# RinceWND/extPOM

Hardware: AMD Instinct MI355X
Metric: 3D cell-updates/sec on internal mode (one internal step = the 3-D baroclinic step and its isplit 2-D external substeps; whole-step wall time) (higher is better)
Workload: dtype f64

## Files before the change

### extpom_amd/csrc/k_vert.hip

```cpp
#include <type_traits>
#include "pomgpu_internal.hpp"
#include "dd_exp.h"

#define dt_(i, j) F2(dt, i, j)
#define dx_(i, j) F2(dx, i, j)
#define dy_(i, j) F2(dy, i, j)
#define h_(i, j) F2(h, i, j)
#define u_(i, j, k) F3(u, i, j, k)
#define v_(i, j, k) F3(v, i, j, k)
#define w_(i, j, k) F3(w, i, j, k)

#define ROWS_PROFUV 1
#define ROWS_PROFT 1
#ifndef ROWS_UVF
#define ROWS_UVF 8
#endif
#ifndef ROWS_UVM
#define ROWS_UVM 4
#endif
#define COL2                               \
  const int i = TID_I, j = TID_J;          \
  if (i > P.iml || j > P.jml) return;

__global__ void k_baropg(KP P, int sum2d) {
// ... 1148 lines not shown
    km_c = km_n;
    if (k + 2 <= kb) km_n = KMA(k + 2);
  }
  const double tps = 0.5 * (F2(cbc, i, j) + F2(cbc, i, j - 1)) *
                     sqrt(sq(.25 * (F3(ub, i, j, kbm1) + F3(ub, i + 1, j, kbm1) + F3(ub, i, j - 1, kbm1) + F3(ub, i + 1, j - 1, kbm1))) +
                          sq(F3(vb, i, j, kbm1)));
  const double c = -P.dti2 * (KMA(kbm1) + P.umol) / (F1(dz, kbm1) * F1(dzz, kbm2) * dh * dh);
  const double m = F2(dvm, i, j);
  double x = (c * gg[kbm2 - 1] - rhs_k) / (tps * P.dti2 / (-F1(dz, kbm1) * dh) - 1. - (ee[kbm2 - 1] - 1.) * c);
  x = x * m;
  F3(vf, i, j, kbm1) = x;
  F2(wvbot, i, j) = -tps * x;
  for (int ki = kbm2; ki >= 1; ki--) {
    x = (ee[ki - 1] * x + gg[ki - 1]) * m;
    F3(vf, i, j, ki) = x;
  }
  if (do_adv) F3(vf, i, j, kb) = 0.;
  F2(tps, i, j) = tps;
#undef RHS
#undef VFLUX
#undef KMA
}

template <int KBT, int V>
static __device__ __forceinline__ void d_profuv_reg(const KP &P, const bool store_tps) {
  const int j = TID_J;
  if (j > P.jm) return;
  int i0, lane = 1;
  if (V) { i0 = TID_I; } else { lane = HALO_LANE; i0 = HALO_COL; }
  const bool out = (lane >= 1 && lane <= 62 && i0 >= 2 && i0 <= P.imm1 && j >= 2 && j <= P.jmm1);
#ifdef POMGPU_EMU
  if (!out) return;
#else
  if (V && !out) return;
  if (j < 2 || j > P.jmm1) return;
#endif
  const int i = i0 < 1 ? 1 : (i0 > P.iml ? P.iml : i0);
  const int iw = i > 1 ? i - 1 : 1, js = j > 1 ? j - 1 : 1;
  const int in_ = V ? i : iw, jn_ = V ? js : j;
  double *f = P.b3 + (size_t)(V ? P3_vf : P3_uf) * P.a3;
  const unsigned col = POMGPU_ST_BYTES * (unsigned)((j - 1) * P.iml + (i - 1)), col2 = POMGPU_ST_BYTES * (unsigned)((js - 1) * P.iml + (i - 1));
  const double *kmp = P.b3 + (size_t)P3_km * P.a3;
#define PLANE(ptr, k, off) REF3((pomgpu_st *)((char *)((pomgpu_st *)(ptr) + (size_t)((k)-1) * P.n2) + (off)), 0)
  const int kb = P.kb, kbm1 = P.kbm1, kbm2 = P.kbm2;
  double ee[KBT], gg[KBT];
#define KC(k) ((k) < kbm1 ? (k) : kbm1)
#define KCB(k) ((k) < kb ? (k) : kb)
#pragma unroll
  for (int k = 1; k <= KBT; k++) ee[k - 1] = PLANE(kmp, KCB(k), col);
  if (V) {
#pragma unroll
    for (int k = 1; k <= KBT; k++) gg[k - 1] = PLANE(kmp, KCB(k), col2);
  } else {
#pragma unroll
    for (int k = 1; k <= KBT - 1; k++) gg[k - 1] = PLANE(f, KC(k), col);
  }
  const double rhs_b = G3(f, i, j, kbm1);
  const double dh = V ? .5 * (F2(h, i, j) + F2(etf, i, j) + F2(h, i, js) + F2(etf, i, js))
                      : (F2(h, i, j) + F2(etf, i, j) + F2(h, iw, j) + F2(etf, iw, j)) * .5;
  const double wsurf = V ? F2(wvsurf, i, j) : F2(wusurf, i, j);
  const double m = V ? F2(dvm, i, j) : F2(dum, i, j);
  const double cb2 = F2(cbc, i, j) + F2(cbc, in_, jn_);
  double tps;
  if (V) tps = 0.5 * cb2 * sqrt(sq(.25 * (F3(ub, i, j, kbm1) + F3(ub, i + 1, j, kbm1) + F3(ub, i, js, kbm1) + F3(ub, i + 1, js, kbm1))) +
                                sq(F3(vb, i, j, kbm1)));
  else tps = 0.5 * cb2 * sqrt(sq(F3(ub, i, j, kbm1)) +
                              sq(.25 * (F3(vb, i, j, kbm1) + F3(vb, i, j + 1, kbm1) + F3(vb, iw, j, kbm1) + F3(vb, iw, j + 1, kbm1))));
  SCHED_FENCE();
#pragma unroll
  for (int k = 1; k <= KBT; k++) {
    ee[k - 1] = (ee[k - 1] + (V ? gg[k - 1] : halo_w(ee[k - 1], [&] { return F3(km, iw, j, KCB(k)); }))) * .5;
    if (!V && (k & 3) == 0) SCHED_FENCE();
  }
  if (V) {
    SCHED_FENCE();
#pragma unroll
    for (int k = 1; k <= KBT - 1; k++) gg[k - 1] = PLANE(f, KC(k), col);
  }
  SCHED_FENCE();
#define KMA(k) ee[(k)-1]
  double km_c = KMA(1), km_n = KMA(2);
  double e_prev, g_prev;
  {
    const double a = -P.dti2 * (km_n + P.umol) / (F1(dz, 1) * F1(dzz, 1) * dh * dh);
    e_prev = a / (a - 1.);
    g_prev = (-P.dti2 * wsurf / (-F1(dz, 1) * dh) - gg[0]) / (a - 1.);
    ee[0] = e_prev; gg[0] = g_prev;
  }
  double e_last = e_prev, g_last = g_prev, km_last = km_n;
#pragma unroll
  for (int k = 2; k <= KBT - 2; k++) {
    km_c = km_n;
    km_n = KMA(k + 1);
    const double a = -P.dti2 * (km_n + P.umol) / (F1(dz, KC(k)) * F1(dzz, KC(k)) * dh * dh);
    const double c = -P.dti2 * (km_c + P.umol) / (F1(dz, KC(k)) * F1(dzz, KC(k - 1)) * dh * dh);
    const double g = 1. / (a + c * (1. - e_prev) - 1.);
    e_prev = a * g;
    g_prev = (c * g_prev - gg[k - 1]) * g;
    ee[k - 1] = e_prev; gg[k - 1] = g_prev;
    const bool fin = (k == kbm2);
    e_last = fin ? e_prev : e_last;
    g_last = fin ? g_prev : g_last;
    km_last = fin ? km_n : km_last;
  }
#undef KMA
  if (!out) return;
  const double c = -P.dti2 * (km_last + P.umol) / (F1(dz, kbm1) * F1(dzz, kbm2) * dh * dh);
  double x = (c * g_last - rhs_b) / (tps * P.dti2 / (-F1(dz, kbm1) * dh) - 1. - (e_last - 1.) * c);
  x = x * m;
  G3(f, i, j, kbm1) = x;
  if (V) F2(wvbot, i, j) = -tps * x; else F2(wubot, i, j) = -tps * x;
#pragma unroll
  for (int ki = KBT - 2; ki >= 1; ki--) {
    const double xn = (ee[ki - 1] * x + gg[ki - 1]) * m;
    if (ki <= kbm2) { x = xn; PLANE(f, ki, col) = x; }
  }
  if (store_tps) F2(tps, i, j) = tps;
#undef KC
#undef KCB
#undef PLANE
}
template <int KBT, int V>
__global__ void __launch_bounds__(64 * ROWS_PROFUV) k_profuv_reg(KP P) { d_profuv_reg<KBT, V>(P, true); }
template <int KBT>
__global__ void __launch_bounds__(64 * ROWS_PROFUV) k_profuv_reg2(KP P) {
  if (blockIdx.z == 0) d_profuv_reg<KBT, 0>(P, false);
  else d_profuv_reg<KBT, 1>(P, true);
}

#define UVF_GHOST(P, i, j) (((i) == 1 && !(P).W) || ((i) == (P).im && !(P).E) || ((j) == 1 && !(P).S) || ((j) == (P).jm && !(P).N))
__global__ void k_uv_filter(KP P, int own) {
  COL2
  if (own && UVF_GHOST(P, i, j)) return;
  const bool act = (i <= P.im && j <= P.jm);
  double su = 0., sv = 0.;
  if (act) {
    for (int k = 1; k <= P.kbm1; k++) {
      const double dzk = F1(dz, k);
      su = su + (F3(uf, i, j, k) + F3(ub, i, j, k) - 2. * F3(u, i, j, k)) * dzk;
      sv = sv + (F3(vf, i, j, k) + F3(vb, i, j, k) - 2. * F3(v, i, j, k)) * dzk;
    }
  }
  for (int k = 1; k <= P.kb; k++) {
    const double uf = F3(uf, i, j, k), vf = F3(vf, i, j, k);
    double u = F3(u, i, j, k), v = F3(v, i, j, k);
    if (act && k <= P.kbm1) {
      u = u + .5 * P.smoth * (uf + F3(ub, i, j, k) - 2. * u - su);
      v = v + .5 * P.smoth * (vf + F3(vb, i, j, k) - 2. * v - sv);
    }
    F3(ub, i, j, k) = u;
// ... 73 lines not shown
        dk[k - 1] = d;
        if (k <= kbm1) {
          su = su + d * F1(dz, k);
          G3(c, i, j, k) = uf;
        }
      }
    }
    SCHED_FENCE();
  }
#pragma unroll
  for (int k = 1; k <= NL; k++)
    if (k <= kbm1) G3(b, i, j, k) = uo[k - 1] + .5 * P.smoth * (dk[k - 1] - su);
  G3(b, i, j, kb) = c_kb;
  G3(c, i, j, kb) = f_kb;
  if (V) F2(tps, i, j) = su;
#undef KC
}
template <int KBT, int V>
__global__ void __launch_bounds__(64 * ROWS_UVF) k_uv_filter_reg(KP P, int own) { d_uv_filter_reg<KBT, V>(P, own); }
template <int KBT>
__global__ void __launch_bounds__(64 * ROWS_UVF) k_uv_filter_reg2(KP P, int own) {
  if (blockIdx.z == 0) d_uv_filter_reg<KBT, 0>(P, own);
  else d_uv_filter_reg<KBT, 1>(P, own);
}

static inline dim3 colblk() { return dim3(64, 2, 1); }
static inline dim3 rowblk(int rows) { return dim3(64, rows, 1); }
static inline dim3 rowgrid(const KP &P, int rows) { return dim3((P.iml + 63) / 64, (P.jml + rows - 1) / rows, 1); }
static inline dim3 colgrid(const KP &P) { return dim3((P.iml + 63) / 64, (P.jml + 1) / 2, 1); }
#define COLV_G(P) dim3(((P).iml + 63) / 64, ((P).jml + 3) / 4, 1)
#define COLV_B dim3(64, 4, 1)
void launch_baropg(pomgpu_ctx *c, int sum2d) {
  if (SW(c, BAROPG_CELLS)) { LAUNCH(c, k_baropg, COLV_G(c->P), COLV_B, c->P, sum2d); return; }
  LAUNCHN(c, "k_baropg", k_baropg_rs, grid1_halo_r(c->P, BPG_ROWS), blk_col_r(BPG_ROWS), c->P, sum2d);
}
void launch_baropg_mcc(pomgpu_ctx *c, int sum2d) { LAUNCH(c, k_baropg_mcc, colgrid(c->P), colblk(), c->P, sum2d); }
void launch_order_pack(pomgpu_ctx *c, double *send_e, double *send_n) {
  const KP &P = c->P;
  const int len = P.iml > P.jml ? P.iml : P.jml;
  LAUNCH(c, k_order_pack, dim3((len + 63) / 64, P.kb + 1, 1), dim3(64, 1, 1), c->P, send_e, send_n);
}
static inline dim3 twin(dim3 g) { g.z = 2; return g; }
template <int KBT> static void launch_int_uvmean_reg_t(pomgpu_ctx *c) {
  if (!SW(c, NO_TWIN)) { LAUNCHN(c, "k_int_uvmean_reg2", (k_int_uvmean_reg2<KBT>), twin(rowgrid(c->P, ROWS_UVM)), rowblk(ROWS_UVM), c->P); return; }
  LAUNCHN(c, "k_int_uvmean_reg", (k_int_uvmean_reg<KBT, 0>), rowgrid(c->P, ROWS_UVM), rowblk(ROWS_UVM), c->P);
  LAUNCHN(c, "k_int_uvmean_reg", (k_int_uvmean_reg<KBT, 1>), rowgrid(c->P, ROWS_UVM), rowblk(ROWS_UVM), c->P);
// ... 76 lines not shown
void launch_advu_profu(pomgpu_ctx *c, int do_adv, int do_prof) { LAUNCH(c, k_advu_profu, colgrid(c->P), colblk(), c->P, do_adv, do_prof); }
void launch_advv_profv(pomgpu_ctx *c, int do_adv, int do_prof) { LAUNCH(c, k_advv_profv, colgrid(c->P), colblk(), c->P, do_adv, do_prof); }
template <int KBT> static void launch_profuv_reg_t(pomgpu_ctx *c) {
  const KP &P = c->P;
  if (!SW(c, NO_TWIN)) {
    LAUNCHN(c, "k_profuv_reg2", (k_profuv_reg2<KBT>), dim3((P.iml + 61) / 62, (P.jml + ROWS_PROFUV - 1) / ROWS_PROFUV, 2), rowblk(ROWS_PROFUV), c->P);
    return;
  }
  LAUNCHN(c, "k_profu_reg", (k_profuv_reg<KBT, 0>), dim3((P.iml + 61) / 62, (P.jml + ROWS_PROFUV - 1) / ROWS_PROFUV, 1), rowblk(ROWS_PROFUV), c->P);
  LAUNCHN(c, "k_profv_reg", (k_profuv_reg<KBT, 1>), rowgrid(P, ROWS_PROFUV), rowblk(ROWS_PROFUV), c->P);
}
int launch_profuv_reg(pomgpu_ctx *c) {
  const int kb = c->P.kb;
  if (SW(c, THOMAS_SCRATCH) || kb > 64 || kb < 6) return 0;
  if (kb <= 24) launch_profuv_reg_t<24>(c);
  else if (kb <= 32) launch_profuv_reg_t<32>(c);
  else if (kb <= 40) launch_profuv_reg_t<40>(c);
  else if (kb <= 44) launch_profuv_reg_t<44>(c);
  else if (kb <= 50) launch_profuv_reg_t<50>(c);
  else if (kb <= 56) launch_profuv_reg_t<56>(c);
  else launch_profuv_reg_t<64>(c);
  return 1;
}
template <int KBT> static void launch_uv_filter_reg_t(pomgpu_ctx *c, int own) {
  if (!SW(c, NO_TWIN)) { LAUNCHN(c, "k_uv_filter_reg2", (k_uv_filter_reg2<KBT>), twin(rowgrid(c->P, ROWS_UVF)), rowblk(ROWS_UVF), c->P, own); return; }
  LAUNCHN(c, "k_uv_filter_reg", (k_uv_filter_reg<KBT, 0>), rowgrid(c->P, ROWS_UVF), rowblk(ROWS_UVF), c->P, own);
  LAUNCHN(c, "k_uv_filter_reg", (k_uv_filter_reg<KBT, 1>), rowgrid(c->P, ROWS_UVF), rowblk(ROWS_UVF), c->P, own);
}
static int launch_uv_filter_reg(pomgpu_ctx *c, int own) {
  const int kb = c->P.kb;
  if (SW(c, THOMAS_SCRATCH) || kb > 64 || kb < 6) return 0;
  if (kb <= 24) launch_uv_filter_reg_t<24>(c, own);
  else if (kb <= 32) launch_uv_filter_reg_t<32>(c, own);
  else if (kb <= 40) launch_uv_filter_reg_t<40>(c, own);
  else if (kb <= 44) launch_uv_filter_reg_t<44>(c, own);
  else if (kb <= 50) launch_uv_filter_reg_t<50>(c, own);
  else if (kb <= 56) launch_uv_filter_reg_t<56>(c, own);
  else launch_uv_filter_reg_t<64>(c, own);
  return 1;
}
void launch_uv_filter(pomgpu_ctx *c, int own) {
  if (launch_uv_filter_reg(c, own)) return;
  LAUNCH(c, k_uv_filter, colgrid(c->P), colblk(), c->P, own);
}
```

### extpom_amd/csrc/pomgpu_api.hip

```cpp
#include <math.h>
#include <stdarg.h>
#include <stdio.h>
#include <stdlib.h>
#include <string.h>
#include <vector>
#include "pomgpu.h"
#include "pomgpu_internal.hpp"

struct ProfPair { int slot; hipEvent_t a, b; };
struct ProfState { std::vector<ProfPair> pending; std::vector<ProfPair> free_; char filter[64]; };
static ProfState *PS(pomgpu_ctx *c) { return (ProfState *)c->prof_state; }

#define SLOT2(c, n) ((c)->P.b2 + (size_t)(n) * (c)->P.n2)
#define SLOT3(c, n) ((c)->P.b3 + (size_t)(n) * (c)->P.a3)
#define D2(c, name) SLOT2(c, P2_##name)
#define D3(c, name) SLOT3(c, P3_##name)
#define LEV3(c, p, lev) ((double *)((pomgpu_st *)(p) + (size_t)(lev) * (c)->P.n2))

int pomgpu_fail(pomgpu_ctx *c, int code, const char *fmt, ...) {
  if (c && c->parent) c = c->parent;
  if (c) {
    va_list ap;
    va_start(ap, fmt);
    vsnprintf(c->err, sizeof c->err, fmt, ap);
// ... 177 lines not shown
static void ext_buffers(pomgpu_ctx *c) {
  KP &P = c->P;
  for (int n = 0; n < POMGPU_NGEN; n++) P.x2[n] = P.y2[n] = c->ext_parity ? c->alt2[n] : P.b2 + (size_t)X2_SLOT[n] * P.n2;
}
static void rho_materialize(pomgpu_ctx *c) {
  if (!c->rho_rt_pending || (c->flags & POMGPU_CTX_2D)) return;
  c->rho_rt_pending = 0;
  launch_roundtrip(c, SLOT3(c, P3_rho), SLOT3(c, P3_rmean), 2);
}
static void side_join(pomgpu_ctx *c);
static void side_begin(pomgpu_ctx *c);
static void side_end(pomgpu_ctx *c, hipEvent_t ev);
static int rim_side(pomgpu_ctx *c);
static void early_invalidate(pomgpu_ctx *c);
void pomgpu_wr_materialize(pomgpu_ctx *c) {
  if (!c->wr_pending) return;
  c->wr_pending = 0;
  (void)hipSetDevice(c->device);
  if (!(c->flags & POMGPU_CTX_2D)) launch_realvertvl(c, 1);
}
static bool wr_on_demand(const pomgpu_ctx *c) {
  return !c->exch && !c->tp.on && !c->wide.on && !c->parent && !(c->flags & POMGPU_CTX_2D) && !c->wr_eager && !SW(c, WR_NODEFER);
}
static void restore_materialize(pomgpu_ctx *c) {
  side_join(c);
  rho_materialize(c);
  pomgpu_wr_materialize(c);
  if (!c->rst_pending) return;
  c->rst_pending = 0;
  launch_restore_fields(c, c->rst_fold, c->rst_fnew);
}
static void ext_flush_deferred(pomgpu_ctx *c);
static void ext_canonical(pomgpu_ctx *c) {
  ext_flush_deferred(c);
  if (!c->ext_parity) return;
  KP &P = c->P;
  for (int n = 0; n < POMGPU_NGEN; n++) launch_copy2(c, P.b2 + (size_t)X2_SLOT[n] * P.n2, c->alt2[n]);
  c->ext_parity = 0;
  ext_buffers(c);
}
static int ctx_create(pomgpu_ctx **out, const pomgpu_dims *d, int device, void *stream, int flags);
extern "C" int pomgpu_create(pomgpu_ctx **out, const pomgpu_dims *d, int device, void *stream) {
  return ctx_create(out, d, device, stream, 0);
}
static int ctx_create(pomgpu_ctx **out, const pomgpu_dims *d, int device, void *stream, int flags) {
  if (!out || !d) return POMGPU_EINVAL;
  *out = NULL;
  if (d->kb < 4 || d->kb > POMGPU_KBMAX || d->im < 5 || d->jm < 5 || d->im > d->im_local || d->jm > d->jm_local) {
    fprintf(stderr, "pomgpu_create: unsupported extents im=%d jm=%d kb=%d (need im,jm>=5, 4<=kb<=%d)\n", d->im, d->jm,
            d->kb, POMGPU_KBMAX);
// ... 38 lines not shown
  c->con.error_status = 0;
  if (stream) { c->stream = (hipStream_t)stream; c->own_stream = false; }
  else {
    if (hipStreamCreateWithFlags(&c->stream, hipStreamNonBlocking) != hipSuccess) { free(c); return POMGPU_EHIP; }
    c->own_stream = true;
  }
  c->cur = c->stream;
  c->prof_state = new ProfState();
  PS(c)->filter[0] = 0;
  bool ok = true;
  auto alloc = [&](double **p, size_t n) {
    if (!ok) return;
    if (hipMalloc((void **)p, n * sizeof(double)) != hipSuccess) { ok = false; *p = NULL; return; }
    if (hipMemsetAsync(*p, 0, n * sizeof(double), c->stream) != hipSuccess) ok = false;
  };
  alloc(&P.b1, (size_t)POM_NBLK1D * P.kb);
  alloc(&P.r1, (size_t)POM_NBLK1D * P.kb);
  alloc(&P.b2, (size_t)POM_NBLK2D * P.n2);
  const bool only2d = (flags & POMGPU_CTX_2D) != 0;
  if (!only2d) alloc(&P.b3, (size_t)POM_NBLK3D * P.a3);
  alloc(&P.bd, nbd);
  for (int n = 0; n < POMGPU_NSCR3 && !only2d; n++) alloc(&P.s3[n], P.n3);
  for (int n = 0; n < POMGPU_NSCR2; n++) alloc(&P.s2[n], P.n2);
  for (int n = 0; n < POMGPU_NCOEF2; n++) alloc(&P.c2[n], P.n2);
  alloc(&c->alt2[0], (size_t)POMGPU_NGEN * P.n2);
  for (int n = 1; n < POMGPU_NGEN && ok; n++) c->alt2[n] = c->alt2[0] + (size_t)n * P.n2;
  { double *m = NULL; alloc(&m, (P.n2 + 7) / 8 + 1); P.m8 = (unsigned char *)m; }
  for (int n = 0; n < 2; n++) {
    const size_t len = (size_t)(P.kb + 1) * (n == 0 ? P.jml : P.iml);
    alloc(&c->ord_send[n], len);
    alloc(&c->ord_recv[n], len);
  }
  if (ok) { P.g4[2] = c->ord_recv[0]; P.g4[0] = c->ord_recv[0] + P.jml; P.g4[3] = c->ord_recv[1]; P.g4[1] = c->ord_recv[1] + P.iml; }
  alloc(&c->d_vel, 4);
  alloc(&c->d_stats, 8);
  if (ok && hipMalloc((void **)&c->d_err, sizeof(int)) != hipSuccess) ok = false;
  if (ok && hipMalloc((void **)&c->d_areas, sizeof(int)) != hipSuccess) ok = false;
  if (ok && hipMemsetAsync(c->d_areas, 0, sizeof(int), c->stream) != hipSuccess) ok = false;
  if (ok && hipMemsetAsync(c->d_err, 0, sizeof(int), c->stream) != hipSuccess) ok = false;
  if (SW(c, DEBUG_ALLOC))
    fprintf(stderr, "pomgpu_create: b1 %p r1 %p b2 %p b3 %p bd %p s3[0] %p s3[4] %p s2[0] %p c2[0] %p\n", (void *)P.b1, (void *)P.r1, (void *)P.b2,
            (void *)P.b3, (void *)P.bd, (void *)P.s3[0], (void *)P.s3[4], (void *)P.s2[0], (void *)P.c2[0]);
  if (!ok) {
    fprintf(stderr, "pomgpu_create: device allocation failed (%zu MB per 3-D array)\n", P.n3 * 8 >> 20);
    pomgpu_destroy(c);
    return POMGPU_ENOMEM;
// ... 7 lines not shown
}

static void wide_free(pomgpu_ctx *c);
extern "C" void pomgpu_destroy(pomgpu_ctx *c) {
  if (!c) return;
  (void)hipSetDevice(c->device);
  if (c->stream) (void)hipStreamSynchronize(c->stream);
  if (c->side) (void)hipStreamSynchronize(c->side);
  if (pomgpu_io_wait(c) != POMGPU_OK)
    fprintf(stderr, "pomgpu_destroy: the output / restart file still being written could not be completed -- call pomgpu_io_wait (or pomgpu_sync) "
                    "before pomgpu_destroy to get its status\n");
  wide_free(c);
  pomgpu_tp_free(c);
  KP &P = c->P;
  (void)hipFree(P.r1);
  if (c->tune_block) {
    (void)hipFree(c->tune_block);
    c->tune_block = NULL; P.b3 = NULL;
    for (int n = 0; n < POMGPU_NSCR3; n++) P.s3[n] = NULL;
  }
  (void)hipFree(P.b1); (void)hipFree(P.b2); (void)hipFree(P.b3); (void)hipFree(P.bd);
  for (int n = 0; n < POMGPU_NSCR3; n++) (void)hipFree(P.s3[n]);
  for (int n = 0; n < POMGPU_NSCR2; n++) (void)hipFree(P.s2[n]);
  for (int n = 0; n < POMGPU_NCOEF2; n++) (void)hipFree(P.c2[n]);
  (void)hipFree(c->alt2[0]); (void)hipFree(c->alt3[0]);
  (void)hipFree(P.m8);
  for (int n = 0; n < 2; n++) { (void)hipFree(c->ord_send[n]); (void)hipFree(c->ord_recv[n]); }
  for (int n = 0; n <= POMGPU_MAXREC; n++) { (void)hipFree(c->rec_t[n]); (void)hipFree(c->rec_s[n]); }
  (void)hipFree(c->d_vel); (void)hipFree(c->d_err); (void)hipFree(c->d_areas); (void)hipFree(c->d_stats); (void)hipFree(c->ext_bar);
  for (int k = 0; k < 3; k++) for (int sl = 0; sl < 4; sl++) { (void)hipFree(c->frc_dev[k][sl][0]); (void)hipFree(c->frc_dev[k][sl][1]); }
  for (int sl = 0; sl < 4; sl++) (void)hipFree(c->lat_dev[sl]);
  ProfState *ps = PS(c);
  if (ps) {
    for (auto &p : ps->pending) { (void)hipEventDestroy(p.a); (void)hipEventDestroy(p.b); }
    for (auto &p : ps->free_) { (void)hipEventDestroy(p.a); (void)hipEventDestroy(p.b); }
    delete ps;
  }
  if (c->side) {
    (void)hipEventDestroy(c->ev_fork); (void)hipEventDestroy(c->ev_early); (void)hipEventDestroy(c->ev_side);
    (void)hipEventDestroy(c->ev_r1); (void)hipEventDestroy(c->ev_r2); (void)hipEventDestroy(c->ev_r8);
    (void)hipEventDestroy(c->ev_rw); (void)hipEventDestroy(c->ev_rq); (void)hipEventDestroy(c->ev_rts);
    (void)hipStreamDestroy(c->side);
  }
  if (c->own_stream && c->stream) (void)hipStreamDestroy(c->stream);
  free(c);
}
// ... 1020 lines not shown
  const KP &P = c->P;
  if (c->side_pending) { (void)hipStreamWaitEvent(c->stream, c->ev_side, 0); c->side_pending = 0; }
  side_begin(c);
  if (with_kernel) launch_realvertvl(c);
  double *arr[1] = {D3(c, wr)};
  const int nz[1] = {P.kbm1};
  const size_t len[8] = {(size_t)P.jm, (size_t)P.jm, (size_t)P.im, (size_t)P.im, 1, 1, 1, 1};
  size_t cnt[8];
  for (int d = 0; d < 8; d++) cnt[d] = c->tp.nbr[d] >= 0 ? (size_t)P.kbm1 * len[d] : 0;
  int rcw = launch_halo_pack8(c, arr, nz, 1, c->tp.send2) ? fail(c, POMGPU_EINVAL, "wr exchange: bad array list") : POMGPU_OK;
  if (!rcw) rcw = pomgpu_tp_move_side(c, cnt, cnt);
  if (!rcw) (void)launch_halo_unpack8(c, arr, nz, 1, (const double *const *)c->tp.recv2);
  side_end(c, c->ev_side);
  c->side_pending = 1;
  return rcw;
}
static int mode_internal(pomgpu_ctx *c, int defer_wr) {
  NEED_HOT(c);
  KP &P = c->P;
  const pom_blkcon &k = c->con;
  rim_wait_r2(c);
  rim_wait_r8(c);
  if ((k.iint != 1 || k.time0 != 0.) && k.mode != 2) {
    launch_int_uvmean(c);
    launch_vertvl(c, 1);
    const bool lib_x = c->tp.on && c->exch;
    const bool rimr = lib_x && rim_side(c) && !SW(c, RIM_RESULTS_MAIN) && !SW(c, UV_FULL_EXCHANGE) && !SW(c, ADVQ_EXCHANGE) && !SW(c, PROD_FULL);
    if (rimr) {
      double *aw[1] = {D3(c, w)};
      const int nw[1] = {P.kb};
      side_begin(c);
      const int rcw = rim_exchange(c, aw, nw, 1);
      side_end(c, c->ev_rw);
      c->rw_pending = 1;
      if (rcw) return rcw;
    }
    else if (!lib_x) xch(c, 1, D3(c, w), P.kb);
    launch_coef_eta(c);
    if (!c->exch || !SW(c, ADVQ_EXCHANGE)) {
      if (SW(c, ADVQ_SINGLE)) {
        launch_advq_col(c, D3(c, q2), D3(c, q2b), D3(c, uf), 1);
        launch_advq_col(c, D3(c, q2l), D3(c, q2lb), D3(c, vf), 1);
      } else {
        launch_advq2_col(c, D3(c, q2), D3(c, q2b), D3(c, uf), D3(c, q2l), D3(c, q2lb), D3(c, vf), 1);
      }
    } else {
// ... 47 lines not shown
      if (!rts) rim_wait_rq(c);
      if (!launch_proft2(c, D3(c, uf), D2(c, wtsurf), D2(c, tsurf), k.nbct, D3(c, vf), D2(c, wssurf), D2(c, ssurf), k.nbcs)) {
        launch_proft(c, D3(c, uf), D2(c, wtsurf), D2(c, tsurf), k.nbct);
        launch_proft(c, D3(c, vf), D2(c, wssurf), D2(c, ssurf), k.nbcs);
      }
      launch_bcond4_edges(c);
      double fold, fnew;
      int rc = restore_prepare(c, &fold, &fnew);
      if (rc) return rc;
      launch_ts_update(c, fold, fnew, k.nadv == 2, 0);
      c->rho_rt_pending = 0;
      c->rst_pending = 1; c->rst_fold = fold; c->rst_fnew = fnew;
      if (rts) {
        double *at[5] = {D3(c, t), D3(c, tb), D3(c, s), D3(c, sb), D3(c, rho)};
        const int nt[5] = {P.kb, P.kb, P.kb, P.kb, P.kb};
        side_begin(c);
        const int rct = rim_exchange(c, at, nt, 5);
        side_end(c, c->ev_rts);
        c->rts_pending = 1;
        if (rct) return rct;
      }
    }
    rim_wait_rq(c);
    if (c->P.kb >= 6 && c->P.kb <= 64 && !SW(c, THOMAS_SCRATCH)) {
      launch_advuv_col(c);
      launch_profuv_reg(c);
    } else {
      launch_advu_profu(c, 1, 1);
      launch_advv_profv(c, 1, 1);
    }
    if (!lib_x) xch(c, 2, D2(c, wubot), 1, D2(c, wvbot), 1);
    launch_bcondorl3(c);
    const bool rim78 = lib_x && !SW(c, UV_FULL_EXCHANGE) && rim_side(c);
    if (rim78) {
      const int top = P.kb - 1;
      double *a7[4] = {D2(c, wubot), D2(c, wvbot), D3(c, uf), D3(c, vf)}, *b7[4] = {D2(c, wubot), D2(c, wvbot), D3(c, u), D3(c, v)};
      const int n7[4] = {1, 1, P.kbm1, P.kbm1};
      side_begin(c);
      int rcs = rim_exchange(c, a7, n7, 4, b7);
      side_end(c, c->ev_r8);
      launch_uv_filter(c, 1);
      double *a8[6] = {D3(c, ub), D3(c, vb), LEV3(c, D3(c, u), top), LEV3(c, D3(c, uf), top), LEV3(c, D3(c, v), top), LEV3(c, D3(c, vf), top)};
      const int n8[6] = {P.kb, P.kb, 1, 1, 1, 1};
      side_begin(c);
      if (!rcs) rcs = rim_exchange(c, a8, n8, 6);
      side_end(c, c->ev_r8);
      c->r8_pending = 1;
      if (rcs) return rcs;
    } else {
      if (lib_x) xch(c, 4, D2(c, wubot), 1, D2(c, wvbot), 1, D3(c, uf), P.kbm1, D3(c, vf), P.kbm1);
      else xch(c, 2, D3(c, uf), P.kbm1, D3(c, vf), P.kbm1);
      launch_uv_filter(c);
      if (lib_x && !SW(c, UV_FULL_EXCHANGE)) {
        const int top = P.kb - 1;
        xch(c, 6, D3(c, ub), P.kb, D3(c, vb), P.kb, LEV3(c, D3(c, u), top), 1, LEV3(c, D3(c, uf), top), 1, LEV3(c, D3(c, v), top), 1, LEV3(c, D3(c, vf), top), 1);
      } else {
        xch(c, 6, D3(c, ub), P.kb, D3(c, u), P.kb, D3(c, uf), P.kb, D3(c, vb), P.kb, D3(c, v), P.kb, D3(c, vf), P.kb);
      }
    }
  }
  launch_int_tail(c);
  const bool side_wr = c->tp.on && c->exch && c->wide.split && c->tp.wr_side;
  if (side_wr && defer_wr && c->wide.on && !SW(c, WR_NODEFER)) {
    c->wr_deferred = 1;
    return POMGPU_OK;
  }
  if (wr_on_demand(c)) { c->wr_pending = 1; return POMGPU_OK; }
  c->wr_pending = 0;
  rim_wait_r8(c);
  launch_realvertvl(c);
  if (side_wr) return wr_on_side(c, 0);
  xch(c, 1, D3(c, wr), P.kbm1);
  return POMGPU_OK;
}
extern "C" int pomgpu_mode_internal(pomgpu_ctx *c) { return mode_internal(c, 0); }
// ... 405 lines not shown
```

### extpom_amd/csrc/pomgpu_internal.hpp

```cpp
#pragma once
#include <hip/hip_runtime.h>
#include <stddef.h>
#include <stdlib.h>
#include "pom_layout.h"

#ifndef COL_ROWS
#define COL_ROWS 4
#endif
#ifndef COL_WX
#define COL_WX 1
#endif
#define POMGPU_NSCR3 8
#define POMGPU_NSCR2 8
#define POMGPU_NCOEF2 24
#define POMGPU_MAXREC 8
#define POMGPU_KBMAX 128
#define POMGPU_CTX_2D 1
#define POMGPU_DERR_VELOCITY 1
#define POMGPU_DERR_BARRIER 2
#define POMGPU_NGEN 7

struct KP {
  int im, jm, kb, imm1, jmm1, kbm1, kbm2, iml, jml;
  int W, E, S, N;
// ... 337 lines not shown
  const int j = by__ * ROWS__ + (int)threadIdx.y / COL_WX + 1;
static inline dim3 grid1_halo_r(const KP &P, int rows) {
  const int nwx = (P.iml + 61) / 62, nbx = (nwx + COL_WX - 1) / COL_WX, nby = (P.jml + rows - 1) / rows, rpx = (nby + 7) / 8;
  if (P.g_lin && 10 * nby < 72 * rpx) return dim3((unsigned)(8 * ((nby * nbx + 7) / 8)), 1, 1);
  return dim3((unsigned)(8 * rpx * nbx), 1, 1);
}
static inline dim3 grid1_halo(const KP &P) { return grid1_halo_r(P, COL_ROWS); }
static inline dim3 blk_col_r(int rows) { return dim3(64, rows * COL_WX, 1); }
static inline dim3 blk_col() { return dim3(64, COL_ROWS * COL_WX, 1); }
#define HALO_COL (int)(((blockIdx.x * blockDim.x + threadIdx.x) >> 6) * 62 + ((blockIdx.x * blockDim.x + threadIdx.x) & 63))
static inline dim3 grid2_halo(const KP &P) { return dim3((P.iml + 61) / 62, (P.jml + 3) / 4, 1); }

#define TID_I (int)(blockIdx.x * blockDim.x + threadIdx.x + 1)
#define TID_J (int)(blockIdx.y * blockDim.y + threadIdx.y + 1)
#define TID_K (int)(blockIdx.z * blockDim.z + threadIdx.z + 1)

#define POMGPU_SWITCHES(X)                                                                                                    \
  X(THOMAS_SCRATCH) X(NO_PAIR) X(EXT_SPLIT) X(ADVAVE_SEPARATE) X(EXT_RIM_KERNEL) X(EXT_LOOP) X(EXT_NOMARCH) X(EXT_MARCH)      \
  X(EXT_ROWS) X(EXT_NOPAIR) X(EXT_PAIR) X(EXT_ROWS2) X(EXT_TWO_SETS) X(EXT_AREAS_LOAD) X(BAROPG_CELLS) X(VERTVL_CELLS)        \
  X(NO_LIN) X(ADVQ_SINGLE) X(ADVT2_SINGLE) X(REALVERTVL_CELLS) X(RHO_ROUNDTRIP) X(TAU_ARRAYS) X(PROFQ_ROWS8) X(PROFQ_ROWS2)    \
  X(PROFQ_NOPACE) X(COL_STRIP) X(BAND_BYTES) X(PAD3) X(IO_SYNC) X(ADVCT_SPLIT) X(ADVQ_EXCHANGE) X(PROD_FULL) X(QFILTER_SPLIT) \
  X(UV_FULL_EXCHANGE) X(NO_OVERLAP) X(NO_SIDE_COMM) X(WR_MAIN) X(WIDE_W) X(WIDE_FULL) X(DEBUG_ALLOC) X(TEST_SPLIT_FAIL_RANK)  \
  X(EDGE_SPLIT) X(WR_NODEFER) X(EXT_RING_FIRST) X(TUNE_FORCE) X(NO_TWIN) X(RIM_MAIN) X(RIM_RESULTS_MAIN) X(SUM2D_OFF) X(ADVCT_ROWS4) X(ADVCT_ROWS8) \
  X(IO_CHUNK_KB)
enum pomgpu_sw {
#define POMGPU_SW_(name) SW_##name,
  POMGPU_SWITCHES(POMGPU_SW_)
#undef POMGPU_SW_
  SW__count
};
struct pomgpu_switches {
  unsigned char on[SW__count];
  long val[SW__count];
};
static const char *const POMGPU_SW_NAMES[SW__count] = {
#define POMGPU_SW_(name) #name,
  POMGPU_SWITCHES(POMGPU_SW_)
#undef POMGPU_SW_
};
static inline void pomgpu_switches_read(pomgpu_switches &s) {
  for (int n = 0; n < SW__count; n++) {
    char var[64] = "POMGPU_";
    size_t k = 7;
    for (const char *q = POMGPU_SW_NAMES[n]; *q && k + 1 < sizeof var; q++) var[k++] = *q;
    var[k] = 0;
    const char *e = getenv(var);
    s.on[n] = e ? 1 : 0;
// ... 65 lines not shown
  int dev3_handed;
  int broken;
  int wr_deferred;
  int side_pending;
  pom_blkcon con;
  int lramp;
  double *rec_t[POMGPU_MAXREC + 1], *rec_s[POMGPU_MAXREC + 1];
  const double *host2, *host3;
  void (*exch)(void *, double *const *, const int *, int);
  void *exch_user;
  void (*order)(void *, const double *, int, const double *, int, double *, double *);
  void *order_user;
  double *ord_send[2], *ord_recv[2];
  double *alt2[POMGPU_NGEN];
  double *alt3[POMGPU_NGEN];
  int ext_parity;
  int ext_deferred;
  int tau_known[2];
  double tau_val[2];
  int rho_rt_pending;
  int rst_pending;
  double rst_fold, rst_fnew;
  int wr_pending;
  int wr_eager;
  double *d_vel;
  int *d_err;
  int *d_areas;
  int areas_checked;
  double *d_stats;
  double *frc_dev[3][4][2];
  int frc_n[3][4];
  double *lat_dev[4];
  int lat_n[4];
  int frc_on, lat_on;
  bool prof_on;
  ProfEntry prof[96];
  int nprof;
  void *prof_state;
  pomgpu_transport tp;
  pomgpu_wide wide;
  pomgpu_ctx *parent;
  int flags;
  unsigned *ext_bar;
  unsigned ext_bar_base;
  int ext_loop_off;
  void *io_job;
// ... 53 lines not shown
    long best = -1, bslots = 0;
    for (long r = 4; r <= rows; r += 4) {
      const long nb = (P.jml + r - 1) / r, slots = (nb + 7) / 8 * 8 * r;
      if (best < 0 || slots < bslots || (slots == bslots && r > best)) { best = r; bslots = slots; }
    }
    P.g_rb = (int)best;
    P.g_bpl = P.g_nbx * (int)(best / 4);
  }
}

void launch_advave_a(pomgpu_ctx *c);
void launch_advave_b(pomgpu_ctx *c);
void launch_advave_c(pomgpu_ctx *c);
void launch_advave_fused(pomgpu_ctx *c);
void launch_advct_col(pomgpu_ctx *c, int sum2d);
void launch_advct_edge(pomgpu_ctx *c, double *to_e, double *to_n);
void launch_advct_fix(pomgpu_ctx *c, const double *from_w, const double *from_s);
void launch_advct_fix2d(pomgpu_ctx *c, int west, int south);
void launch_advt2x2_col(pomgpu_ctx *c, const double *tb, const double *t, const double *tc, double *tf, const double *sb, const double *s_,
                        const double *sc, double *sf);
void launch_advq2_col(pomgpu_ctx *c, const double *q, const double *qb, double *qf, const double *ql, const double *qlb, double *qlf, int zero_else);
void launch_advuv_col(pomgpu_ctx *c);
int launch_profuv_reg(pomgpu_ctx *c);
void launch_advave_m2a(pomgpu_ctx *c);
void launch_advave_m2b(pomgpu_ctx *c);
void launch_vint(pomgpu_ctx *c, int only_aam, int ghost = 0);
void launch_modeint_tail(pomgpu_ctx *c);
void launch_ext_elf(pomgpu_ctx *c);
void launch_ext_uvaf(pomgpu_ctx *c, int interior);
void launch_ext_update(pomgpu_ctx *c);
void launch_ext_step(pomgpu_ctx *c, const KP &Q, int store_f, int fuse_adv);
void launch_check_areas(pomgpu_ctx *c);
int launch_ext_loop(pomgpu_ctx *c, const KP &Q, int first, int last);
int launch_ext_pair_ok(const pomgpu_switches &sw, const KP &Q);
int launch_ext_pair(pomgpu_ctx *c, const KP &Q, double *const *T, int store_f2);
void launch_copy2(pomgpu_ctx *c, double *dst, const double *src);
void launch_lat(pomgpu_ctx *c, int phase, const double *rec, double fold, double fnew);
void launch_frc_load(pomgpu_ctx *c, const double *ra, const double *rb, double *xf, double *yf);
void launch_frc_interp(pomgpu_ctx *c, double fold, double fnew, double *x, const double *xb, const double *xf, double *y, const double *yb,
                       const double *yf);
void launch_int_tail(pomgpu_ctx *c);
void launch_bcond1(pomgpu_ctx *c);
void launch_advct_a(pomgpu_ctx *c);
void launch_advct_b(pomgpu_ctx *c);
void launch_advct_c(pomgpu_ctx *c);
void launch_aam(pomgpu_ctx *c);
// ... 67 lines not shown
```

Baseline: 4.171 billion.

## Fuse vertical u/v diffusion solve with time filter for interior columns

When the run is single-GPU and unpartitioned, the implicit vertical friction solve for u and v now applies the Asselin time filter in the same kernel for interior columns. It writes the filtered ub/ub-shift results directly instead of storing uf/vf and rereading them in a separate filter kernel. A small rim kernel handles the edge columns, and the bottom-level ub/vb values are snapshotted first so the in-place update does not race with neighbouring reads. The copy of uf/vf for the interior is deferred and only materialized on demand, which saves a full 3-D read/write pass per step but adds extra launches, register pressure and complexity around ordering.

```diff
diff --git a/extpom_amd/csrc/k_vert.hip b/extpom_amd/csrc/k_vert.hip
--- a/extpom_amd/csrc/k_vert.hip
+++ b/extpom_amd/csrc/k_vert.hip
@@ -1194,8 +1194,8 @@
 #undef KMA
 }
 
-template <int KBT, int V>
-static __device__ __forceinline__ void d_profuv_reg(const KP &P, const bool store_tps) {
+template <int KBT, int V, int FUSE = 0>
+static __device__ __forceinline__ void d_profuv_reg(const KP &P, const bool store_tps, const double *ubk = nullptr, const double *vbk = nullptr) {
   const int j = TID_J;
   if (j > P.jm) return;
   int i0, lane = 1;
@@ -1234,10 +1234,14 @@
   const double m = V ? F2(dvm, i, j) : F2(dum, i, j);
   const double cb2 = F2(cbc, i, j) + F2(cbc, in_, jn_);
   double tps;
-  if (V) tps = 0.5 * cb2 * sqrt(sq(.25 * (F3(ub, i, j, kbm1) + F3(ub, i + 1, j, kbm1) + F3(ub, i, js, kbm1) + F3(ub, i + 1, js, kbm1))) +
-                                sq(F3(vb, i, j, kbm1)));
-  else tps = 0.5 * cb2 * sqrt(sq(F3(ub, i, j, kbm1)) +
-                              sq(.25 * (F3(vb, i, j, kbm1) + F3(vb, i, j + 1, kbm1) + F3(vb, iw, j, kbm1) + F3(vb, iw, j + 1, kbm1))));
+#define UBK(i, j) (FUSE ? G2(ubk, i, j) : (double)F3(ub, i, j, kbm1))
+#define VBK(i, j) (FUSE ? G2(vbk, i, j) : (double)F3(vb, i, j, kbm1))
+  if (V) tps = 0.5 * cb2 * sqrt(sq(.25 * (UBK(i, j) + UBK(i + 1, j) + UBK(i, js) + UBK(i + 1, js))) +
+                                sq(VBK(i, j)));
+  else tps = 0.5 * cb2 * sqrt(sq(UBK(i, j)) +
+                              sq(.25 * (VBK(i, j) + VBK(i, j + 1) + VBK(iw, j) + VBK(iw, j + 1))));
+#undef UBK
+#undef VBK
   SCHED_FENCE();
 #pragma unroll
   for (int k = 1; k <= KBT; k++) {
@@ -1280,14 +1284,69 @@
   const double c = -P.dti2 * (km_last + P.umol) / (F1(dz, kbm1) * F1(dzz, kbm2) * dh * dh);
   double x = (c * g_last - rhs_b) / (tps * P.dti2 / (-F1(dz, kbm1) * dh) - 1. - (e_last - 1.) * c);
   x = x * m;
-  G3(f, i, j, kbm1) = x;
-  if (V) F2(wvbot, i, j) = -tps * x; else F2(wubot, i, j) = -tps * x;
-#pragma unroll
-  for (int ki = KBT - 2; ki >= 1; ki--) {
-    const double xn = (ee[ki - 1] * x + gg[ki - 1]) * m;
-    if (ki <= kbm2) { x = xn; PLANE(f, ki, col) = x; }
-  }
-  if (store_tps) F2(tps, i, j) = tps;
+  if (!FUSE) {
+    G3(f, i, j, kbm1) = x;
+    if (V) F2(wvbot, i, j) = -tps * x; else F2(wubot, i, j) = -tps * x;
+#pragma unroll
+    for (int ki = KBT - 2; ki >= 1; ki--) {
+      const double xn = (ee[ki - 1] * x + gg[ki - 1]) * m;
+      if (ki <= kbm2) { x = xn; PLANE(f, ki, col) = x; }
+    }
+    if (store_tps) F2(tps, i, j) = tps;
+  } else {
+    if (V) F2(wvbot, i, j) = -tps * x; else F2(wubot, i, j) = -tps * x;
+    const bool inner = (i >= 5 && i <= P.im - 3 && j >= 5 && j <= P.jm - 3);
+    const unsigned o_in = inner ? col : BOFF_NONE, o_fr = inner ? BOFF_NONE : col;
+    const unsigned lvb = LVB;
+    const BufA bf = BUF3(f), bb = BUF3(P.b3 + (size_t)(V ? P3_vb : P3_ub) * P.a3), bc = BUF3(P.b3 + (size_t)(V ? P3_v : P3_u) * P.a3);
+#define LVK(k) ((unsigned)(KC(k) - 1) * lvb)
+#pragma unroll
+    for (int ki = KBT - 1; ki >= 1; ki--) {
+      if (ki <= KBT - 2) {
+        const double xn = (ee[ki - 1] * x + gg[ki - 1]) * m;
+        x = (ki <= kbm2) ? xn : x;
+      }
+      bst(bf, o_fr, LVK(ki), x);
+      ee[ki - 1] = (double)(pomgpu_st)x;
+      gg[ki - 1] = bld(bc, o_in, LVK(ki));
+    }
+    constexpr int CH = 8, NL = KBT - 1, NCH = (NL + CH - 1) / CH;
+    double t0[CH], t1[CH];
+#pragma unroll
+    for (int q = 0; q < CH; q++) t0[q] = bld(bb, o_in, LVK(q + 1));
+    const double c_kb = bld(bc, o_in, (unsigned)(kb - 1) * lvb), f_kb = bld(bf, o_in, (unsigned)(kb - 1) * lvb);
+    double su = 0.;
+#pragma unroll
+    for (int ch = 0; ch < NCH; ch++) {
+      if (ch + 1 < NCH) {
+#pragma unroll
+        for (int q = 0; q < CH; q++) {
+          const double y = bld(bb, o_in, LVK((ch + 1) * CH + q + 1));
+          if (ch & 1) t0[q] = y; else t1[q] = y;
+        }
+      }
+      SCHED_FENCE();
+#pragma unroll
+      for (int q = 0; q < CH; q++) {
+        const int k = ch * CH + q + 1;
+        if (k <= NL) {
+          const double uf = ee[k - 1];
+          const double d = uf + ((ch & 1) ? t1[q] : t0[q]) - 2. * gg[k - 1];
+          ee[k - 1] = d;
+          const double sn = su + d * F1(dz, KC(k));
+          su = (k <= kbm1) ? sn : su;
+          bst(bc, o_in, LVK(k), uf);
+        }
+      }
+      SCHED_FENCE();
+    }
+#pragma unroll
+    for (int k = 1; k <= NL; k++) bst(bb, o_in, LVK(k), gg[k - 1] + .5 * P.smoth * (ee[k - 1] - su));
+    bst(bb, o_in, (unsigned)(kb - 1) * lvb, c_kb);
+    bst(bc, o_in, (unsigned)(kb - 1) * lvb, f_kb);
+    if (store_tps) F2(tps, i, j) = inner ? su : tps;
+#undef LVK
+  }
 #undef KC
 #undef KCB
 #undef PLANE
@@ -1298,6 +1357,23 @@
 __global__ void __launch_bounds__(64 * ROWS_PROFUV) k_profuv_reg2(KP P) {
   if (blockIdx.z == 0) d_profuv_reg<KBT, 0>(P, false);
   else d_profuv_reg<KBT, 1>(P, true);
+}
+
+template <int KBT>
+__global__ void __launch_bounds__(64 * ROWS_PROFUV) k_profuv_filter_reg2(KP P, const double *ubk, const double *vbk) {
+  if (blockIdx.z == 0) d_profuv_reg<KBT, 0, 1>(P, false, ubk, vbk);
+  else d_profuv_reg<KBT, 1, 1>(P, true, ubk, vbk);
+}
+__global__ void k_uvb_bottom(KP P, double *ubk, double *vbk) {
+  const int i = TID_I, j = TID_J;
+  if (i > P.iml || j > P.jml) return;
+  G2(ubk, i, j) = F3(ub, i, j, P.kbm1);
+  G2(vbk, i, j) = F3(vb, i, j, P.kbm1);
+}
+__global__ void k_uvf_copy(KP P, double *dst, const double *src) {
+  const int i = TID_I + 4, j = TID_J + 4, k = TID_K;
+  if (i > P.im - 3 || j > P.jm - 3 || k > P.kbm1) return;
+  G3(dst, i, j, k) = G3(src, i, j, k);
 }
 
 #define UVF_GHOST(P, i, j) (((i) == 1 && !(P).W) || ((i) == (P).im && !(P).E) || ((j) == 1 && !(P).S) || ((j) == (P).jm && !(P).N))
@@ -1417,6 +1493,55 @@
 __global__ void __launch_bounds__(64 * ROWS_UVF) k_uv_filter_reg2(KP P, int own) {
   if (blockIdx.z == 0) d_uv_filter_reg<KBT, 0>(P, own);
   else d_uv_filter_reg<KBT, 1>(P, own);
+}
+
+template <int V>
+static __device__ __forceinline__ void d_uv_filter_rim(const KP &P) {
+  const int t = (int)(blockIdx.x * blockDim.x + threadIdx.x), line = (int)blockIdx.y;
+  int i, j;
+  if (line == 0) {
+    const int il = t & 7;
+    j = (t >> 3) + 1;
+    if (il == 7 || j > P.jm) return;
+    i = il < 4 ? il + 1 : P.im - 6 + il;
+  } else {
+    i = t + 5;
+    if (i > P.im - 3) return;
+    j = line <= 4 ? line : P.jm - 7 + line;
+  }
+  const double *f = P.b3 + (size_t)(V ? P3_vf : P3_uf) * P.a3;
+  double *b = P.b3 + (size_t)(V ? P3_vb : P3_ub) * P.a3, *c = P.b3 + (size_t)(V ? P3_v : P3_u) * P.a3;
+  const int kb = P.kb, kbm1 = P.kbm1;
+  constexpr int CH = 8;
+  double xf[CH], xb[CH], xc[CH];
+#define KC(k) ((k) < kbm1 ? (k) : kbm1)
+  double su = 0.;
+  for (int k0 = 1; k0 <= kbm1; k0 += CH) {
+#pragma unroll
+    for (int q = 0; q < CH; q++) { xf[q] = G3(f, i, j, KC(k0 + q)); xb[q] = G3(b, i, j, KC(k0 + q)); xc[q] = G3(c, i, j, KC(k0 + q)); }
+#pragma unroll
+    for (int q = 0; q < CH; q++)
+      if (k0 + q <= kbm1) su = su + (xf[q] + xb[q] - 2. * xc[q]) * F1(dz, k0 + q);
+  }
+  for (int k0 = 1; k0 <= kbm1; k0 += CH) {
+#pragma unroll
+    for (int q = 0; q < CH; q++) { xf[q] = G3(f, i, j, KC(k0 + q)); xb[q] = G3(b, i, j, KC(k0 + q)); xc[q] = G3(c, i, j, KC(k0 + q)); }
+#pragma unroll
+    for (int q = 0; q < CH; q++)
+      if (k0 + q <= kbm1) {
+        G3(b, i, j, k0 + q) = xc[q] + .5 * P.smoth * ((xf[q] + xb[q] - 2. * xc[q]) - su);
+        G3(c, i, j, k0 + q) = xf[q];
+      }
+  }
+  const double c_kb = G3(c, i, j, kb), f_kb = G3(f, i, j, kb);
+  G3(b, i, j, kb) = c_kb;
+  G3(c, i, j, kb) = f_kb;
+  if (V) F2(tps, i, j) = su;
+#undef KC
+}
+__global__ void k_uv_filter_rim(KP P) {
+  if (blockIdx.z == 0) d_uv_filter_rim<0>(P);
+  else d_uv_filter_rim<1>(P);
 }
 
 static inline dim3 colblk() { return dim3(64, 2, 1); }
@@ -1539,6 +1664,33 @@
   else launch_profuv_reg_t<64>(c);
   return 1;
 }
+template <int KBT> static void launch_profuv_filter_reg_t(pomgpu_ctx *c, double *ubk, double *vbk) {
+  const KP &P = c->P;
+  LAUNCH(c, k_uvb_bottom, grid2(P), blk2(), c->P, ubk, vbk);
+  LAUNCHN(c, "k_profuv_filter_reg2", (k_profuv_filter_reg2<KBT>), dim3((P.iml + 61) / 62, (P.jml + ROWS_PROFUV - 1) / ROWS_PROFUV, 2), rowblk(ROWS_PROFUV), c->P,
+          (const double *)ubk, (const double *)vbk);
+}
+void launch_profuv_filter_reg(pomgpu_ctx *c, double *ubk, double *vbk) {
+  const int kb = c->P.kb;
+  if (kb <= 24) launch_profuv_filter_reg_t<24>(c, ubk, vbk);
+  else if (kb <= 32) launch_profuv_filter_reg_t<32>(c, ubk, vbk);
+  else if (kb <= 40) launch_profuv_filter_reg_t<40>(c, ubk, vbk);
+  else if (kb <= 44) launch_profuv_filter_reg_t<44>(c, ubk, vbk);
+  else if (kb <= 50) launch_profuv_filter_reg_t<50>(c, ubk, vbk);
+  else if (kb <= 56) launch_profuv_filter_reg_t<56>(c, ubk, vbk);
+  else launch_profuv_filter_reg_t<64>(c, ubk, vbk);
+}
+void launch_uv_filter_rim(pomgpu_ctx *c) {
+  const KP &P = c->P;
+  const int len = 8 * P.jm > P.im - 7 ? 8 * P.jm : P.im - 7;
+  LAUNCH(c, k_uv_filter_rim, dim3((len + 63) / 64, 8, 2), dim3(64, 1, 1), c->P);
+}
+void launch_uvf_copy(pomgpu_ctx *c) {
+  const KP &P = c->P;
+  const dim3 g((P.im - 7 + 63) / 64, (P.jm - 7 + 3) / 4, P.kbm1);
+  LAUNCH(c, k_uvf_copy, g, blk2(), c->P, P.b3 + (size_t)P3_uf * P.a3, (const double *)(P.b3 + (size_t)P3_u * P.a3));
+  LAUNCH(c, k_uvf_copy, g, blk2(), c->P, P.b3 + (size_t)P3_vf * P.a3, (const double *)(P.b3 + (size_t)P3_v * P.a3));
+}
 template <int KBT> static void launch_uv_filter_reg_t(pomgpu_ctx *c, int own) {
   if (!SW(c, NO_TWIN)) { LAUNCHN(c, "k_uv_filter_reg2", (k_uv_filter_reg2<KBT>), twin(rowgrid(c->P, ROWS_UVF)), rowblk(ROWS_UVF), c->P, own); return; }
   LAUNCHN(c, "k_uv_filter_reg", (k_uv_filter_reg<KBT, 0>), rowgrid(c->P, ROWS_UVF), rowblk(ROWS_UVF), c->P, own);
diff --git a/extpom_amd/csrc/pomgpu_api.hip b/extpom_amd/csrc/pomgpu_api.hip
--- a/extpom_amd/csrc/pomgpu_api.hip
+++ b/extpom_amd/csrc/pomgpu_api.hip
@@ -223,10 +223,21 @@
 static bool wr_on_demand(const pomgpu_ctx *c) {
   return !c->exch && !c->tp.on && !c->wide.on && !c->parent && !(c->flags & POMGPU_CTX_2D) && !c->wr_eager && !SW(c, WR_NODEFER);
 }
+static bool uv_fused(const pomgpu_ctx *c) {
+  const KP &P = c->P;
+  return !c->exch && !c->tp.on && !c->wide.on && !c->parent && !(c->flags & POMGPU_CTX_2D) && !c->wr_eager && P.kb >= 6 && P.kb <= 64 &&
+         P.im >= 8 && P.jm >= 8 && !SW(c, THOMAS_SCRATCH) && !SW(c, NO_TWIN) && !SW(c, UV_NOFUSE);
+}
+static void uvf_materialize(pomgpu_ctx *c) {
+  if (!c->uvf_pending) return;
+  c->uvf_pending = 0;
+  launch_uvf_copy(c);
+}
 static void restore_materialize(pomgpu_ctx *c) {
   side_join(c);
   rho_materialize(c);
   pomgpu_wr_materialize(c);
+  uvf_materialize(c);
   if (!c->rst_pending) return;
   c->rst_pending = 0;
   launch_restore_fields(c, c->rst_fold, c->rst_fnew);
@@ -311,6 +322,7 @@
   alloc(&P.bd, nbd);
   for (int n = 0; n < POMGPU_NSCR3 && !only2d; n++) alloc(&P.s3[n], P.n3);
   for (int n = 0; n < POMGPU_NSCR2; n++) alloc(&P.s2[n], P.n2);
+  for (int n = 0; n < 2 && !only2d; n++) alloc(&c->uvb_bot[n], P.n2);
   for (int n = 0; n < POMGPU_NCOEF2; n++) alloc(&P.c2[n], P.n2);
   alloc(&c->alt2[0], (size_t)POMGPU_NGEN * P.n2);
   for (int n = 1; n < POMGPU_NGEN && ok; n++) c->alt2[n] = c->alt2[0] + (size_t)n * P.n2;
@@ -364,6 +376,7 @@
   (void)hipFree(P.b1); (void)hipFree(P.b2); (void)hipFree(P.b3); (void)hipFree(P.bd);
   for (int n = 0; n < POMGPU_NSCR3; n++) (void)hipFree(P.s3[n]);
   for (int n = 0; n < POMGPU_NSCR2; n++) (void)hipFree(P.s2[n]);
+  (void)hipFree(c->uvb_bot[0]); (void)hipFree(c->uvb_bot[1]);
   for (int n = 0; n < POMGPU_NCOEF2; n++) (void)hipFree(P.c2[n]);
   (void)hipFree(c->alt2[0]); (void)hipFree(c->alt3[0]);
   (void)hipFree(P.m8);
@@ -1430,6 +1443,7 @@
   rim_wait_r2(c);
   rim_wait_r8(c);
   if ((k.iint != 1 || k.time0 != 0.) && k.mode != 2) {
+    c->uvf_pending = 0;
     launch_int_uvmean(c);
     launch_vertvl(c, 1);
     const bool lib_x = c->tp.on && c->exch;
@@ -1523,9 +1537,11 @@
       }
     }
     rim_wait_rq(c);
+    const bool fuse = uv_fused(c);
     if (c->P.kb >= 6 && c->P.kb <= 64 && !SW(c, THOMAS_SCRATCH)) {
       launch_advuv_col(c);
-      launch_profuv_reg(c);
+      if (fuse) launch_profuv_filter_reg(c, c->uvb_bot[0], c->uvb_bot[1]);
+      else launch_profuv_reg(c);
     } else {
       launch_advu_profu(c, 1, 1);
       launch_advv_profv(c, 1, 1);
@@ -1551,7 +1567,8 @@
     } else {
       if (lib_x) xch(c, 4, D2(c, wubot), 1, D2(c, wvbot), 1, D3(c, uf), P.kbm1, D3(c, vf), P.kbm1);
       else xch(c, 2, D3(c, uf), P.kbm1, D3(c, vf), P.kbm1);
-      launch_uv_filter(c);
+      if (fuse) { launch_uv_filter_rim(c); c->uvf_pending = 1; }
+      else launch_uv_filter(c);
       if (lib_x && !SW(c, UV_FULL_EXCHANGE)) {
         const int top = P.kb - 1;
         xch(c, 6, D3(c, ub), P.kb, D3(c, vb), P.kb, LEV3(c, D3(c, u), top), 1, LEV3(c, D3(c, uf), top), 1, LEV3(c, D3(c, v), top), 1, LEV3(c, D3(c, vf), top), 1);
diff --git a/extpom_amd/csrc/pomgpu_internal.hpp b/extpom_amd/csrc/pomgpu_internal.hpp
--- a/extpom_amd/csrc/pomgpu_internal.hpp
+++ b/extpom_amd/csrc/pomgpu_internal.hpp
@@ -383,7 +383,7 @@
   X(PROFQ_NOPACE) X(COL_STRIP) X(BAND_BYTES) X(PAD3) X(IO_SYNC) X(ADVCT_SPLIT) X(ADVQ_EXCHANGE) X(PROD_FULL) X(QFILTER_SPLIT) \
   X(UV_FULL_EXCHANGE) X(NO_OVERLAP) X(NO_SIDE_COMM) X(WR_MAIN) X(WIDE_W) X(WIDE_FULL) X(DEBUG_ALLOC) X(TEST_SPLIT_FAIL_RANK)  \
   X(EDGE_SPLIT) X(WR_NODEFER) X(EXT_RING_FIRST) X(TUNE_FORCE) X(NO_TWIN) X(RIM_MAIN) X(RIM_RESULTS_MAIN) X(SUM2D_OFF) X(ADVCT_ROWS4) X(ADVCT_ROWS8) \
-  X(IO_CHUNK_KB)
+  X(IO_CHUNK_KB) X(UV_NOFUSE)
 enum pomgpu_sw {
 #define POMGPU_SW_(name) SW_##name,
   POMGPU_SWITCHES(POMGPU_SW_)
@@ -495,6 +495,8 @@
   int rst_pending;
   double rst_fold, rst_fnew;
   int wr_pending;
+  int uvf_pending;
+  double *uvb_bot[2];
   int wr_eager;
   double *d_vel;
   int *d_err;
@@ -594,6 +596,9 @@
 void launch_advq2_col(pomgpu_ctx *c, const double *q, const double *qb, double *qf, const double *ql, const double *qlb, double *qlf, int zero_else);
 void launch_advuv_col(pomgpu_ctx *c);
 int launch_profuv_reg(pomgpu_ctx *c);
+void launch_profuv_filter_reg(pomgpu_ctx *c, double *ubk, double *vbk);
+void launch_uv_filter_rim(pomgpu_ctx *c);
+void launch_uvf_copy(pomgpu_ctx *c);
 void launch_advave_m2a(pomgpu_ctx *c);
 void launch_advave_m2b(pomgpu_ctx *c);
 void launch_vint(pomgpu_ctx *c, int only_aam, int ghost = 0);
```

After: 4.239 billion, median of 6. 1.02x the previous value.
